# NagabhushanSN95/SimpleNeRF

Hardware: AMD Instinct MI355X
Metric: rays/sec (coarse+fine, 128+128 samples) (higher is better)
Workload: dtype f32; 1 GPU; headline: 1024 rays/GPU x (128 coarse + 128 fine -> 256 merged) samples, 8x256 coarse+fine MLPs, LLFF fern NDC rays, eval; rays_per_gpu=1024, samples=128+128, parallelism=ray-shard x1

## Files before the change

### simplenerf_amd/csrc/mlp_backward.hip

```cpp
#include "mlp_generic.h"
#include <algorithm>
#include <type_traits>

#include "mlp_device_f16.h"

namespace snerf {
int mlp_backward_chain_f16x3(const MlpPlan& plan, const ChainArgs& a, int products, hipStream_t stream);
int mlp_backward_chain_bf16(const MlpPlan& plan, const ChainArgs& a, hipStream_t stream);
}

namespace {

template <int U>
__device__ __forceinline__ void zero_acc(f32x16 (&acc)[U]) {
#pragma unroll
    for (int u = 0; u < U; ++u)
#pragma unroll
        for (int r = 0; r < 16; ++r) acc[u][r] = 0.0f;
}

template <int U>
__device__ __forceinline__ void load_relu_words(unsigned (&words)[U / 2], const unsigned* __restrict__ masks, int t0, int lane) {
#pragma unroll
    for (int p = 0; p < U / 2; ++p) words[p] = __builtin_nontemporal_load(masks + ((t0 >> 1) + p) * 64 + lane);
}
template <int U>
__device__ __forceinline__ void relu_backward(const f32x16 (&acc)[U], const unsigned (&words)[U / 2], float (&dy)[U * 16]) {
#pragma unroll
    for (int u = 0; u < U; u += 2)
#pragma unroll
        for (int r = 0; r < 32; ++r) dy[16 * u + r] = keep_if_bit(acc[u + (r >> 4)][r & 15], words[u >> 1], r);
}

template <int WT, int VT, bool VIEWDEP>
__global__ void __launch_bounds__(256, 1) mlp_backward_chain_kernel(ChainArgs a) {
    extern __shared__ __attribute__((aligned(16))) float lds[];
    const int lane = threadIdx.x & 63;
    const int wave = __builtin_amdgcn_readfirstlane(threadIdx.x >> 6);
    const int half = lane >> 5;
    SlabStream<WT> st;
    st.start(a.packed + a.dgrad_offset, lds, lane, wave);

    const long long block = (long long)blockIdx.x * 4 + wave;
    const long long first = block * 32 + (lane & 31);
    const bool live = first < a.total;
    const unsigned* masks = reinterpret_cast<const unsigned*>(a.acts + (block * a.act_rows + a.act_mask) * 32);
    float* grads = a.grads + block * a.grad_rows * 32;

    float dhead[4];
    dhead[0] = live && a.sigma[first] > 0.0f ? a.d_sigma[first] : 0.0f;
#pragma unroll
    for (int c = 0; c < 3; ++c) {
        const float col = live ? a.rgb[first * 3 + c] : 0.0f;
        dhead[c + 1] = live ? a.d_rgb[first * 3 + c] * (col * (1.0f - col)) : 0.0f;
    }
    if (half == 0) {
#pragma unroll
        for (int c = 0; c < 4; ++c) grads[(a.grad_head + c) * 32 + (lane & 31)] = dhead[c];
    }

    f32x16 acc[WT];
    zero_acc<WT>(acc);
    float dy[WT * 16];
    if (VIEWDEP) {
        const float* wv = a.packed + a.views_out_w;
        unsigned hv_bits[VT / 2];
#pragma unroll
        for (int p = 0; p < VT / 2; ++p) hv_bits[p] = masks[((a.depth * WT) / 2 + p) * 64 + lane];
        float dyv[VT * 16];
#pragma unroll
        for (int g = 0; g < VT * 4; ++g) {
            f32x4 w0 = *reinterpret_cast<const f32x4*>(wv + 0 * VT * 32 + 8 * g + 4 * half);
            f32x4 w1 = *reinterpret_cast<const f32x4*>(wv + 1 * VT * 32 + 8 * g + 4 * half);
            f32x4 w2 = *reinterpret_cast<const f32x4*>(wv + 2 * VT * 32 + 8 * g + 4 * half);
#pragma unroll
            for (int q = 0; q < 4; ++q) {
                const float v = fmaf(w2[q], dhead[3], fmaf(w1[q], dhead[2], w0[q] * dhead[1]));
                const int n = 4 * g + q;
                dyv[n] = (hv_bits[n >> 5] >> (n & 31)) & 1u ? v : 0.0f;
            }
        }
        store_acc_tile(dyv, grads + a.grad_yv * 32, lane);
        gemm_segment<WT, VT, WT>(acc, dyv, st);
        to_operand<WT, false>(acc, dy);
        store_acc_tile(dy, grads + a.grad_feature * 32, lane);
        zero_acc<WT>(acc);
        gemm_segment<WT, WT, WT>(acc, dy, st);
    }
    {
        const float* wo = a.packed + a.pts_out_w;
#pragma unroll
        for (int g = 0; g < WT * 4; ++g) {
            const f32x4 w0 = *reinterpret_cast<const f32x4*>(wo + 8 * g + 4 * half);
            f32x4 w1 = {0, 0, 0, 0}, w2 = {0, 0, 0, 0}, w3 = {0, 0, 0, 0};
            if (!VIEWDEP) {
                w1 = *reinterpret_cast<const f32x4*>(wo + 1 * WT * 32 + 8 * g + 4 * half);
                w2 = *reinterpret_cast<const f32x4*>(wo + 2 * WT * 32 + 8 * g + 4 * half);
                w3 = *reinterpret_cast<const f32x4*>(wo + 3 * WT * 32 + 8 * g + 4 * half);
            }
#pragma unroll
            for (int q = 0; q < 4; ++q) {
                float v = w0[q] * dhead[0];
                if (!VIEWDEP) v = fmaf(w3[q], dhead[3], fmaf(w2[q], dhead[2], fmaf(w1[q], dhead[1], v)));
                acc[g >> 2][4 * (g & 3) + q] += v;
            }
        }
    }
    unsigned relu_words[WT / 2];
    load_relu_words<WT>(relu_words, masks, (a.depth - 1) * WT, lane);
#pragma unroll 1
    for (int l = a.depth - 1; l >= 0; --l) {
        relu_backward<WT>(acc, relu_words, dy);
        if (l > 0) load_relu_words<WT>(relu_words, masks, (l - 1) * WT, lane);
        store_acc_tile(dy, grads + (l * a.width) * 32, lane);
        if (l == 0) break;
        zero_acc<WT>(acc);
        gemm_segment<WT, WT, WT>(acc, dy, st);
    }
    asm volatile("s_waitcnt vmcnt(0)" ::: "memory");
}

struct WgradJob {
    int dy_row0, out_rows, out_tiles;
    int x_row0, in_rows, in_tiles;
    int grad_rows, act_rows;
    int chunks;
    long long blocks;
    long long partial_off;
    long long bias_off;
    int w_param, w_ld, w_col;
    int b_param;
    int half;
    int dy_skip;
    int x_kind;
    int feat_lo, feat_hi;
    int x8;
    int x2_row0, x2_tiles;
    int launched, partial_ld, partial_col0;
};

__host__ __device__ inline int pe_position_feature(int p, int kind) {
    const int c = p & 15;
    const int n = 8 * (p >> 4) + 4 * (c >> 3) + (c & 3), h = (c >> 2) & 1;
    return snerf::pe_feature(n, h, kind == snerf::SEG_POINTS_PE ? snerf::kPointsPairs : snerf::kViewsPairs, 16);
}

constexpr int kRegionSlots = 64, kRegionWords = 128;
constexpr int kRegionTableFloat0 = 448;
__device__ __forceinline__ float region_max(const float* workspace, int region) {
    const unsigned w = reinterpret_cast<const unsigned*>(workspace)[kRegionTableFloat0 + (threadIdx.x & (kRegionSlots - 1)) * kRegionWords + region];
    float v = __uint_as_float(w);
#pragma unroll
    for (int off = 32; off > 0; off >>= 1) v = fmaxf(v, __shfl_xor(v, off, 64));
    return v;
}

__host__ __device__ inline float wgrad_scale(float max_abs) {
    if (!(max_abs > 0.0f) || !(max_abs < 3.0e38f)) return 1.0f;
    int e;
    frexpf(max_abs, &e);
    int shift = 10 - e;
    if (shift > 120) shift = 120;
    if (shift < -120) shift = -120;
    return ldexpf(1.0f, shift);
}

__device__ __forceinline__ void split_fragment(const float* __restrict__ row, int c0, int swz, float k, f16x8& hi, f16x8& lo,
                                               float& sum) {
    const f32x4 v0 = *reinterpret_cast<const f32x4*>(row + ((c0 ^ swz) << 2));
    const f32x4 v1 = *reinterpret_cast<const f32x4*>(row + (((c0 + 1) ^ swz) << 2));
    sum += (v0[0] + v0[1]) + (v0[2] + v0[3]) + (v1[0] + v1[1]) + (v1[2] + v1[3]);
    typedef float f32x2 __attribute__((ext_vector_type(2)));
    typedef _Float16 f16x2 __attribute__((ext_vector_type(2)));
#pragma unroll
    for (int j = 0; j < 4; j += 2) {
        const f32x2 a = f32x2{v0[j], v0[j + 1]} * k, b = f32x2{v1[j], v1[j + 1]} * k;
        const f16x2 ah = __builtin_convertvector(a, f16x2), bh = __builtin_convertvector(b, f16x2);
        const f16x2 al = __builtin_convertvector(a - __builtin_convertvector(ah, f32x2), f16x2);
        const f16x2 bl = __builtin_convertvector(b - __builtin_convertvector(bh, f32x2), f16x2);
        hi[j] = ah[0]; hi[j + 1] = ah[1]; lo[j] = al[0]; lo[j + 1] = al[1];
        hi[4 + j] = bh[0]; hi[5 + j] = bh[1]; lo[4 + j] = bl[0]; lo[5 + j] = bl[1];
    }
}

__device__ __forceinline__ void lds_dma_16(const float* src, const float* lds_dst) {
    const unsigned base = __builtin_amdgcn_readfirstlane(
        (unsigned)(size_t)(__attribute__((address_space(3))) const void*)lds_dst);
    asm volatile("s_mov_b32 m0, %0\n\ts_nop 0\n\tglobal_load_lds_dwordx4 %1, off nt" ::"s"(base), "v"(src) : "memory", "m0");
}

__device__ __forceinline__ void lds_dma_16_base(const void* uniform_base, unsigned lane_byte_offset, unsigned lds_byte_address) {
    asm volatile("s_mov_b32 m0, %0\n\ts_nop 0\n\tglobal_load_lds_dwordx4 %1, %2 nt" ::"s"(lds_byte_address), "v"(lane_byte_offset),
                 "s"(uniform_base)
                 : "memory", "m0");
}

constexpr int kMaxJobs = 16;
struct JobTable {
    int count;
    int wg_start[kMaxJobs + 1];
    WgradJob jobs[kMaxJobs];
};
struct GradPointers {
    float* p[40];
};

template <int NO, int NI, bool F16>
__global__ void __launch_bounds__(256, 1) wgrad_kernel(JobTable table, const float* __restrict__ grads,
                                                       const float* __restrict__ acts, float* __restrict__ partial,
                                                       const float* __restrict__ zeros) {
    extern __shared__ __attribute__((aligned(16))) float lds[];
    const int tid = threadIdx.x;
    const int lane = tid & 63;
    const int wave = __builtin_amdgcn_readfirstlane(tid >> 6);
    const int half = lane >> 5;
    int ji = 0;
    while (ji + 1 < table.count && (int)blockIdx.x >= table.wg_start[ji + 1]) ++ji;
    const WgradJob& job = table.jobs[ji];
    const int chunk = blockIdx.x - table.wg_start[ji];
    const int rows_dy = job.out_tiles * 32, rows_x = job.in_tiles * 32, rows = rows_dy + rows_x;
    const int wgrid_i = job.in_tiles / NI;
    const int wo = wave / wgrid_i, wi = wave - wo * wgrid_i;
    const bool active = wo * NO < job.out_tiles;
    const long long per = (job.blocks + job.chunks - 1) / job.chunks;
    const long long b0 = chunk * per, b1 = (b0 + per < job.blocks) ? b0 + per : job.blocks;

    f32x16 acc[NO][NI];
    float bsum[NO];
#pragma unroll
    for (int oo = 0; oo < NO; ++oo) {
        bsum[oo] = 0.0f;
#pragma unroll
        for (int ii = 0; ii < NI; ++ii)
#pragma unroll
            for (int r = 0; r < 16; ++r) acc[oo][ii][r] = 0.0f;
    }

    const int buf_floats = rows * 32;
    constexpr int kMaxSlots = 16;
    const int per_wave = rows >> 5;
    const char* slot_src[kMaxSlots];
    int slot_rows[kMaxSlots];
    const char* zero_page = reinterpret_cast<const char*>(zeros + 192);
    const long long dy_stride = (long long)job.grad_rows * 128, x_stride = (long long)job.act_rows * 128;
#pragma unroll
    for (int k = 0; k < kMaxSlots; ++k) {
        const int r0 = (wave + 4 * k) * 8;
        int real;
        const char* src;
        if (r0 < rows_dy) {
            real = job.out_rows - r0;
            src = reinterpret_cast<const char*>(grads) + (b0 * job.grad_rows + job.dy_row0 + r0) * 128;
        } else {
            real = job.in_rows - (r0 - rows_dy);
            src = reinterpret_cast<const char*>(acts) + (b0 * job.act_rows + job.x_row0 + (r0 - rows_dy)) * 128;
        }
        real = real < 0 ? 0 : (real > 8 ? 8 : real);
        slot_rows[k] = real;
        slot_src[k] = real > 0 ? src : zero_page;
    }
    const unsigned lane_off = (lane >> 3) * 128 + (((lane & 7) ^ ((4 * (wave & 1) + (lane >> 4)) & 7)) << 4);
    const unsigned lds_base = (unsigned)(size_t)(__attribute__((address_space(3))) const void*)lds;
    const bool all_full = job.out_rows == rows_dy && job.in_rows == rows_x;
    const int dy_slots = (rows_dy / 8 - wave + 3) >> 2;
    const char* dy_run = reinterpret_cast<const char*>(grads) + (b0 * job.grad_rows + job.dy_row0 + wave * 8) * 128;
    const char* x_run = reinterpret_cast<const char*>(acts) + (b0 * job.act_rows + job.x_row0 + wave * 8 - rows_dy) * 128;
    auto stage_next = [&](int buffer_floats) {
        if (all_full) {
#pragma unroll
            for (int k = 0; k < kMaxSlots; ++k)
                if (k < per_wave)
                    lds_dma_16_base(k < dy_slots ? dy_run : x_run, lane_off + k * 4096,
                                    lds_base + (unsigned)buffer_floats * 4 + (wave + 4 * k) * 1024);
            dy_run += dy_stride;
            x_run += x_stride;
            return;
        }
#pragma unroll
        for (int k = 0; k < kMaxSlots; ++k) {
            if (k < per_wave) {
                const unsigned dst = lds_base + (unsigned)buffer_floats * 4 + (wave + 4 * k) * 1024;
                const int real = slot_rows[k];
                if (real == 8 || real == 0) {
                    lds_dma_16_base(slot_src[k], real ? lane_off : lane * 16, dst);
                } else {
                    const char* p = (lane >> 3) < real ? slot_src[k] + lane_off : zero_page + lane * 16;
                    lds_dma_16(reinterpret_cast<const float*>(p), reinterpret_cast<const float*>(lds) + buffer_floats + (wave + 4 * k) * 256);
                }
                if (real) slot_src[k] += (wave + 4 * k) * 8 < rows_dy ? dy_stride : x_stride;
            }
        }
    };

    const int swz = ((lane & 31) >> 1) & 7;
    const int row_off = (lane & 31) * 32;
    const int a_base = wo * NO * 1024;
    const int b_base = rows_dy * 32 + wi * NI * 1024;

    const float gk = F16 ? wgrad_scale(region_max(zeros, job.dy_row0 / 32)) : 1.0f;
    if constexpr (F16) {
        struct SplitSet {
            f16x8 ah[NO], al[NO], bh[NI], bl[NI];
        };
        auto convert = [&](SplitSet& f, const float* buf, int kk, float counted) {
            const int c0 = 4 * kk + 2 * half;
            float unused = 0.0f;
#pragma unroll
            for (int oo = 0; oo < NO; ++oo) {
                float part = 0.0f;
                split_fragment(buf + a_base + oo * 1024 + row_off, c0, swz, gk, f.ah[oo], f.al[oo], part);
                bsum[oo] += part * counted;
            }
#pragma unroll
            for (int ii = 0; ii < NI; ++ii) split_fragment(buf + b_base + ii * 1024 + row_off, c0, swz, 1.0f, f.bh[ii], f.bl[ii], unused);
        };
        auto products = [&](const SplitSet& f) {
#pragma unroll
            for (int oo = 0; oo < NO; ++oo)
#pragma unroll
                for (int ii = 0; ii < NI; ++ii) {
                    acc[oo][ii] = __builtin_amdgcn_mfma_f32_32x32x16_f16(f.ah[oo], f.bh[ii], acc[oo][ii], 0, 0, 0);
                    acc[oo][ii] = __builtin_amdgcn_mfma_f32_32x32x16_f16(f.ah[oo], f.bl[ii], acc[oo][ii], 0, 0, 0);
                    acc[oo][ii] = __builtin_amdgcn_mfma_f32_32x32x16_f16(f.al[oo], f.bh[ii], acc[oo][ii], 0, 0, 0);
                }
        };
        const int nblocks = (int)(b1 - b0);
        SplitSet even, odd;
        if (nblocks > 0) {
            stage_next(0);
            if (nblocks > 1) stage_next(buf_floats);
            if (nblocks > 1) wait_vmcnt(per_wave < 63 ? per_wave : 63); else asm volatile("s_waitcnt vmcnt(0)" ::: "memory");
            __syncthreads();
            if (active) convert(even, lds, 0, 1.0f);
        }
        for (int n = 0; n < nblocks; ++n) {
            const float* cur = lds + (n & 1) * buf_floats;
            const float* nxt = lds + ((n + 1) & 1) * buf_floats;
            if (active) {
                products(even);
                convert(odd, cur, 1, 1.0f);
            }
            asm volatile("s_waitcnt vmcnt(0) lgkmcnt(0)" ::: "memory");
            __syncthreads();
            if (n + 2 < nblocks) stage_next((n & 1) * buf_floats);
            if (active) {
                products(odd);
                convert(even, n + 1 < nblocks ? nxt : cur, 0, n + 1 < nblocks ? 1.0f : 0.0f);
            }
        }
    } else {
    if (b0 < b1) stage_next(0);
    for (long long b = b0; b < b1; ++b) {
        asm volatile("s_waitcnt vmcnt(0)" ::: "memory");
        __syncthreads();
        const float* cur = lds + ((b - b0) & 1) * buf_floats;
        if (b + 1 < b1) stage_next((int)((b - b0 + 1) & 1) * buf_floats);
        if (active) {
#pragma unroll 1
            for (int g = 0; g < 4; ++g) {
                const int off = (((2 * g + half) ^ swz) << 2) + row_off;
                f32x4 av[NO], bv[NI];
#pragma unroll
                for (int oo = 0; oo < NO; ++oo) av[oo] = *reinterpret_cast<const f32x4*>(cur + a_base + oo * 1024 + off);
#pragma unroll
                for (int ii = 0; ii < NI; ++ii) bv[ii] = *reinterpret_cast<const f32x4*>(cur + b_base + ii * 1024 + off);
#pragma unroll
                for (int oo = 0; oo < NO; ++oo) {
#pragma unroll
                    for (int ii = 0; ii < NI; ++ii)
#pragma unroll
                        for (int q = 0; q < 4; ++q)
                            acc[oo][ii] = __builtin_amdgcn_mfma_f32_32x32x2f32(av[oo][q], bv[ii][q], acc[oo][ii], 0, 0, 0);
                    bsum[oo] += (av[oo][0] + av[oo][1]) + (av[oo][2] + av[oo][3]);
                }
            }
        }
    }
    }
    asm volatile("s_waitcnt vmcnt(0)" ::: "memory");
    if (!active) return;
    const int in_cols = job.in_tiles * 32;
    float* out = partial + job.partial_off + (long long)chunk * rows_dy * in_cols;
    float* bout = partial + job.bias_off + (long long)chunk * rows_dy;
#pragma unroll
    for (int oo = 0; oo < NO; ++oo) {
        const int o = wo * NO + oo;
#pragma unroll
        for (int ii = 0; ii < NI; ++ii) {
            const int i = wi * NI + ii;
#pragma unroll
            for (int r = 0; r < 16; ++r) {
                const int row = (r & 3) + 8 * (r >> 2) + 4 * half;
                out[(long long)(o * 32 + row) * in_cols + i * 32 + (lane & 31)] = acc[oo][ii][r];
            }
        }
        if (wi == 0) {
            const float sum = bsum[oo] + __shfl_xor(bsum[oo], 32, 64);
            if (half == 0) bout[o * 32 + lane] = sum;
        }
    }
}


typedef unsigned u32x2 __attribute__((ext_vector_type(2)));

__device__ __forceinline__ u32x2 lds_read_tr8(unsigned lds_byte_address, int byte_offset) {
    u32x2 v;
    asm volatile("ds_read_b64_tr_b8 %0, %1 offset:%2" : "=v"(v) : "v"(lds_byte_address), "i"(byte_offset) : "memory");
    return v;
}
__device__ __forceinline__ u32x2 lds_read_tr16(unsigned lds_byte_address, int byte_offset) {
    u32x2 v;
    asm volatile("ds_read_b64_tr_b16 %0, %1 offset:%2" : "=v"(v) : "v"(lds_byte_address), "i"(byte_offset) : "memory");
    return v;
}
template <typename T>
__device__ __forceinline__ void after_lds_wait(T& v) {
    asm volatile("" : "+v"(v));
}
union Frag16 {
// ... 805 lines not shown
```

### simplenerf_amd/csrc/mlp_device.h

```cpp
#pragma once
#include "mlp_plan.h"

typedef float f32x16 __attribute__((ext_vector_type(16)));
typedef float f32x4 __attribute__((ext_vector_type(4)));
typedef float f32x2 __attribute__((ext_vector_type(2)));

struct MlpArgs {
    const float* packed;
    const float* origins;
    const float* dirs;
    const float* view_dirs;
    const float* depths;
    const float* noise;
    float* sigma;
    float* rgb;
    long long total;
    int samples;
    int depth;
    int width;
    long long bias_offset, feature_bias, views_bias, pts_out_w, pts_out_b, views_out_w, views_out_b;
    float* acts;
    int act_rows, act_pev, act_h1, act_feature, act_hv, act_mask;
    int const_floats;
    float* visibility;
    const float* view_dirs2;
    float* visibility2;
    int num_other;
    int* range_flag;
    const int* weight_range;
};

struct ChainArgs {
    const float* packed;
    const float* acts;
    const float* sigma;
    const float* rgb;
    const float* d_sigma;
    const float* d_rgb;
    float* grads;
    long long total;
    int depth, width;
    long long dgrad_offset, pts_out_w, views_out_w;
    int act_rows, act_h1, act_hv, act_mask;
    int grad_rows, grad_feature, grad_yv, grad_head;
    unsigned* dy_max;
};

__host__ __device__ inline float renorm_factor(float max_abs) {
    if (!(max_abs > 0.0f) || !(max_abs < 3.0e38f)) return 1.0f;
    int e;
    frexpf(max_abs, &e);
    int shift = 4 - e;
    if (shift > 120) shift = 120;
    if (shift < -120) shift = -120;
    return ldexpf(1.0f, shift);
}

template <int N>
__device__ __forceinline__ void store_acc_tile(const float (&h)[N], float* __restrict__ tile, int lane) {
    const int j = lane & 31, half = lane >> 5;
#pragma unroll
    for (int n = 0; n < N; ++n) {
        const int f = 32 * (n >> 4) + (n & 3) + 8 * ((n & 15) >> 2) + 4 * half;
        __builtin_nontemporal_store(h[n], tile + f * 32 + j);
    }
}
template <int N>
__device__ __forceinline__ void load_acc_tile(float (&h)[N], const float* __restrict__ tile, int lane) {
    const int j = lane & 31, half = lane >> 5;
#pragma unroll
    for (int n = 0; n < N; ++n) {
        const int f = 32 * (n >> 4) + (n & 3) + 8 * ((n & 15) >> 2) + 4 * half;
        h[n] = tile[f * 32 + j];
    }
}
__device__ __forceinline__ float keep_if_bit(float v, unsigned word, int bit) {
    return __uint_as_float(__float_as_uint(v) & (unsigned)__builtin_amdgcn_sbfe((int)word, bit, 1));
}
__device__ __forceinline__ float keep_if_bit_2op(float v, unsigned word, int bit) {
    int k = __builtin_amdgcn_sbfe((int)word, bit, 1);
    asm("" : "+v"(k));
    return __uint_as_float(__float_as_uint(v) & (unsigned)k);
}
__device__ __forceinline__ unsigned positive_bits(unsigned m, float a, float b) {
    const f32x2 t = f32x2{0.0f, 0.0f} - f32x2{a, b};
    m = __builtin_amdgcn_alignbit(m, __float_as_uint(t[0]), 31);
    return __builtin_amdgcn_alignbit(m, __float_as_uint(t[1]), 31);
}
__device__ __forceinline__ unsigned relu_bits(const float* __restrict__ h) {
    unsigned m = 0;
#pragma unroll
    for (int r = 15; r >= 1; r -= 2) m = positive_bits(m, h[r], h[r - 1]);
    return m;
}
template <int N>
__device__ __forceinline__ void store_relu_masks(const float (&h)[N], unsigned* __restrict__ masks, int t0, int lane) {
#pragma unroll
    for (int u = 0; u < N / 16; u += 2)
        __builtin_nontemporal_store(relu_bits(h + 16 * u) | (relu_bits(h + 16 * (u + 1)) << 16), masks + ((t0 + u) >> 1) * 64 + lane);
}
template <int PAIRS, int NREG>
__device__ __forceinline__ void store_pe_tile(const float (&pe)[NREG], float* __restrict__ tile, int lane) {
    const int j = lane & 31, half = lane >> 5;
#pragma unroll
    for (int n = 0; n < NREG; ++n) {
        const int e0 = snerf::pe_feature(n, 0, PAIRS, 16), e1 = snerf::pe_feature(n, 1, PAIRS, 16);
        const int e = half ? e1 : e0;
        if (e >= 0) __builtin_nontemporal_store(pe[n], tile + e * 32 + j);
    }
}

template <int WT>
struct SlabStream {
    static constexpr int kBufFloats = WT * 1024;
    const float* cur;
    float* lds;
    int parity;
    int lane, wave;

    __device__ __forceinline__ void fetch(const float* src, float* dst) const {
#pragma unroll
        for (int i = 0; i < WT; ++i) {
            const int chunk = i * 4 + wave;
            __builtin_amdgcn_global_load_lds((const __attribute__((address_space(1))) void*)(src + chunk * 256 + lane * 4),
                                             (__attribute__((address_space(3))) void*)(dst + chunk * 256), 16, 0, 0);
        }
    }
    __device__ __forceinline__ void start(const float* first, float* lds_base, int lane_, int wave_) {
        cur = first; lds = lds_base; parity = 0; lane = lane_; wave = wave_;
        fetch(cur, lds);
    }
    template <int U>
    __device__ __forceinline__ const float* acquire() {
        asm volatile("s_waitcnt vmcnt(0)" ::: "memory");
        __syncthreads();
        const float* ready = lds + parity * kBufFloats;
        cur += U * 1024;
        parity ^= 1;
        return ready;
    }
    template <int I>
    __device__ __forceinline__ void fetch_piece() const {
        const int chunk = I * 4 + wave;
        __builtin_amdgcn_global_load_lds((const __attribute__((address_space(1))) void*)(cur + chunk * 256 + lane * 4),
                                         (__attribute__((address_space(3))) void*)(lds + parity * kBufFloats + chunk * 256),
                                         16, 0, 0);
    }
};

template <int I, int WT>
__device__ __forceinline__ void fetch_piece_if(const SlabStream<WT>& st) {
    if constexpr (I >= 0 && I < WT) st.template fetch_piece<I>();
}
template <int U, int WT, int EVERY>
__device__ __forceinline__ void constexpr_fetch(const SlabStream<WT>& st, int slot) {
#pragma unroll
    for (int i = 0; i < WT; ++i)
        if (slot == i * EVERY) {
            const int chunk = i * 4 + st.wave;
            __builtin_amdgcn_global_load_lds((const __attribute__((address_space(1))) void*)(st.cur + chunk * 256 + st.lane * 4),
                                             (__attribute__((address_space(3))) void*)(st.lds + st.parity * SlabStream<WT>::kBufFloats + chunk * 256),
                                             16, 0, 0);
        }
}
template <int WT, int DONE>
__device__ __forceinline__ void tail_fetch(const SlabStream<WT>& st) {
#pragma unroll
    for (int i = DONE; i < WT; ++i) {
        const int chunk = i * 4 + st.wave;
        __builtin_amdgcn_global_load_lds((const __attribute__((address_space(1))) void*)(st.cur + chunk * 256 + st.lane * 4),
                                         (__attribute__((address_space(3))) void*)(st.lds + st.parity * SlabStream<WT>::kBufFloats + chunk * 256),
                                         16, 0, 0);
    }
}

template <int U, int NSLAB, int WT, int NB>
__device__ __forceinline__ void gemm_segment(f32x16 (&acc)[U], const float (&b)[NB], SlabStream<WT>& st) {
    static_assert(NB >= NSLAB * 16, "B operand array too short");
    constexpr int kSlots = 4 * U;
    constexpr int kEvery = kSlots >= WT ? kSlots / WT : 1;
#pragma unroll
    for (int sl = 0; sl < NSLAB; ++sl) {
        const float* slab = st.template acquire<U>() + st.lane * 4;
#pragma unroll
        for (int g = 0; g < 4; ++g) {
#pragma unroll
            for (int u = 0; u < U; ++u) {
                const f32x4 a = *reinterpret_cast<const f32x4*>(slab + (g * U + u) * 256);
#pragma unroll
                for (int q = 0; q < 4; ++q)
                    acc[u] = __builtin_amdgcn_mfma_f32_32x32x2f32(a[q], b[sl * 16 + g * 4 + q], acc[u], 0, 0, 0);
                constexpr_fetch<U, WT, kEvery>(st, g * U + u);
            }
        }
        if (kSlots < WT) tail_fetch<WT, kSlots>(st);
    }
}

template <int U, int NB>
__device__ __forceinline__ void gemm_resident_slab(f32x16 (&acc)[U], const float (&b)[NB], const float* slab) {
    static_assert(NB >= 16, "B operand array too short");
#pragma unroll
    for (int g = 0; g < 4; ++g) {
#pragma unroll
        for (int u = 0; u < U; ++u) {
            const f32x4 a = *reinterpret_cast<const f32x4*>(slab + (g * U + u) * 256);
#pragma unroll
            for (int q = 0; q < 4; ++q) acc[u] = __builtin_amdgcn_mfma_f32_32x32x2f32(a[q], b[g * 4 + q], acc[u], 0, 0, 0);
        }
    }
}

template <int U>
__device__ __forceinline__ void load_bias(f32x16 (&acc)[U], const float* __restrict__ bias, int half) {
#pragma unroll
    for (int u = 0; u < U; ++u) {
#pragma unroll
        for (int g = 0; g < 4; ++g) {
            const f32x4 v = *reinterpret_cast<const f32x4*>(bias + 32 * u + 8 * g + 4 * half);
#pragma unroll
            for (int q = 0; q < 4; ++q) acc[u][4 * g + q] = v[q];
        }
    }
}

template <int U, bool RELU>
__device__ __forceinline__ void to_operand(const f32x16 (&acc)[U], float (&h)[U * 16]) {
#pragma unroll
    for (int u = 0; u < U; ++u)
#pragma unroll
        for (int r = 0; r < 16; ++r) h[16 * u + r] = RELU ? fmaxf(acc[u][r], 0.0f) : acc[u][r];
}

template <int N>
__device__ __forceinline__ float head_dot(const float (&h)[N], const float* __restrict__ w, int half) {
    float s = 0.0f;
#pragma unroll
    for (int g = 0; g < N / 4; ++g) {
        const f32x4 v = *reinterpret_cast<const f32x4*>(w + 8 * g + 4 * half);
#pragma unroll
        for (int q = 0; q < 4; ++q) s = fmaf(v[q], h[4 * g + q], s);
    }
    return s + __shfl_xor(s, 32, 64);
}

__device__ __forceinline__ float sigmoidf(float x) { return __fdiv_rn(1.0f, 1.0f + expf(-x)); }

__device__ __forceinline__ f32x2 opaque_pair(float v) {
    f32x2 p = {v, v};
    asm volatile("" : "+v"(p));
    return p;
}

template <bool PAIRED = false>
__device__ __forceinline__ void sincos_turns(double turns, float& s, float& c) {
    const double f = turns - rint(turns);
    const double q = rint(4.0 * f);
    const double g = f - 0.25 * q;
    const float th = (float)(g * 6.283185307179586476925);
    float t2 = th * th, t2c = t2;
    if constexpr (PAIRED) {
        const f32x2 both = opaque_pair(t2);
        t2 = both.x; t2c = both.y;
    }
    float sp = fmaf(t2, 2.7557319e-6f, -1.9841270e-4f);
    sp = fmaf(sp, t2, 8.3333333e-3f);
    sp = fmaf(sp, t2, -1.6666667e-1f);
    sp = fmaf(th * t2, sp, th);
    float cp = fmaf(t2c, -2.7557319e-7f, 2.4801587e-5f);
    cp = fmaf(cp, t2c, -1.3888889e-3f);
    cp = fmaf(cp, t2c, 4.1666667e-2f);
    cp = fmaf(cp, t2c, -0.5f);
    cp = fmaf(cp, t2c, 1.0f);
    const int qi = ((int)q) & 3;
    const float s0 = (qi & 1) ? cp : sp;
    const float c0 = (qi & 1) ? sp : cp;
    s = (qi >= 2) ? -s0 : s0;
    c = (qi == 1 || qi == 2) ? -c0 : c0;
}

template <int PAIRS, int NREG, bool PAIRED = false>
__device__ __forceinline__ void encode(const float (&x)[3], int half, float (&pe)[NREG]) {
    constexpr double kInvTwoPi = 0.15915494309189533576888;
    const double r0 = (double)x[0] * kInvTwoPi, r1 = (double)x[1] * kInvTwoPi, r2 = (double)x[2] * kInvTwoPi;
#pragma unroll
    for (int m = 0; m < PAIRS / 2; ++m) {
        constexpr int dummy = 0;
        (void)dummy;
        const int c0 = 2 * m, c1 = 2 * m + 1;
        const int d0 = c0 % 3, d1 = c1 % 3;
        const double a0 = d0 == 0 ? r0 : (d0 == 1 ? r1 : r2);
        const double a1 = d1 == 0 ? r0 : (d1 == 1 ? r1 : r2);
        const double f0 = (double)(1 << (c0 / 3)), f1 = (double)(1 << (c1 / 3));
        const double turns = half ? a1 * f1 : a0 * f0;
        sincos_turns<PAIRED>(turns, pe[2 * m], pe[2 * m + 1]);
    }
    pe[PAIRS] = half ? x[2] : x[0];
    pe[PAIRS + 1] = half ? 0.0f : x[1];
#pragma unroll
    for (int n = PAIRS + 2; n < NREG; ++n) pe[n] = 0.0f;
}
```

### simplenerf_amd/csrc/mlp_forward_body.h

```cpp
#pragma once
#include "mlp_device.h"

namespace {

template <int WT, int VT, bool VIEWDEP, bool SIGMA_PE, bool STORE, bool VIS = false>
__device__ __forceinline__ void mlp_forward_body(const MlpArgs& a, long long block, float* lds) {
    static_assert(!VIS || VIEWDEP, "the visibility row belongs to the views head");
    const int lane = threadIdx.x & 63;
    const int wave = __builtin_amdgcn_readfirstlane(threadIdx.x >> 6);
    const int half = lane >> 5;

    SlabStream<WT> st;
    st.start(a.packed, lds, lane, wave);
    float* consts = lds + 2 * SlabStream<WT>::kBufFloats;
    for (int i = threadIdx.x * 4; i < a.const_floats; i += 256 * 4)
        *reinterpret_cast<f32x4*>(consts + i) = *reinterpret_cast<const f32x4*>(a.packed + a.bias_offset + i);
    __syncthreads();

    const long long first = (block * 4 + wave) * 32 + (lane & 31);
    const bool live = first < a.total;
    const long long g = live ? first : a.total - 1;
    const long long ray = g / a.samples;
    const float z = a.depths[g];
    float x[3];
#pragma unroll
    for (int k = 0; k < 3; ++k) x[k] = a.origins[ray * 3 + k] + a.dirs[ray * 3 + k] * z;

    float pe[snerf::kPointsKSteps];
    encode<snerf::kPointsPairs, snerf::kPointsKSteps>(x, half, pe);
    float pev[snerf::kViewsKSteps];
    if (VIEWDEP) {
        float v[3];
#pragma unroll
        for (int k = 0; k < 3; ++k) v[k] = a.view_dirs[ray * 3 + k];
        encode<snerf::kViewsPairs, snerf::kViewsKSteps>(v, half, pev);
    }

    float* tile = nullptr;
    unsigned* masks = nullptr;
    if (STORE) {
        tile = a.acts + (block * 4 + wave) * a.act_rows * 32;
        masks = reinterpret_cast<unsigned*>(tile + a.act_mask * 32);
        store_pe_tile<snerf::kPointsPairs, snerf::kPointsKSteps>(pe, tile, lane);
        if (VIEWDEP) store_pe_tile<snerf::kViewsPairs, snerf::kViewsKSteps>(pev, tile + a.act_pev * 32, lane);
    }

    const float* bias = consts;
    f32x16 acc[WT];
    float h[WT * 16];
    load_bias<WT>(acc, bias, half);
    gemm_segment<WT, 2, WT>(acc, pe, st);
    to_operand<WT, true>(acc, h);
    if (STORE) {
        store_acc_tile(h, tile + a.act_h1 * 32, lane);
        store_relu_masks(h, masks, 0, lane);
    }
#pragma unroll 1
    for (int l = 1; l < a.depth; ++l) {
        load_bias<WT>(acc, bias + (long long)l * a.width, half);
        if (l == 5) gemm_segment<WT, 2, WT>(acc, pe, st);
        gemm_segment<WT, WT, WT>(acc, h, st);
        to_operand<WT, true>(acc, h);
        if (STORE) {
            store_acc_tile(h, tile + (a.act_h1 + l * a.width) * 32, lane);
            store_relu_masks(h, masks, l * WT, lane);
        }
    }

    const float* wout = consts + (a.pts_out_w - a.bias_offset);
    const float* bout = consts + (a.pts_out_b - a.bias_offset);
    float sigma = head_dot<WT * 16>(h, wout, half) + bout[0];
    if (a.noise) sigma += a.noise[g];
    sigma = fmaxf(sigma, 0.0f);
    float rgb[3];
    if (!VIEWDEP) {
#pragma unroll
        for (int c = 0; c < 3; ++c) rgb[c] = sigmoidf(head_dot<WT * 16>(h, wout + (c + 1) * WT * 32, half) + bout[c + 1]);
    } else {
        load_bias<WT>(acc, consts + (a.feature_bias - a.bias_offset), half);
        gemm_segment<WT, WT, WT>(acc, h, st);
        to_operand<WT, false>(acc, h);
        if (STORE) store_acc_tile(h, tile + a.act_feature * 32, lane);
        f32x16 accv[VT];
        load_bias<VT>(accv, consts + (a.views_bias - a.bias_offset), half);
        gemm_segment<VT, WT, WT>(accv, h, st);
        if (SIGMA_PE) gemm_segment<VT, 2, WT>(accv, pe, st);
        f32x16 accv_base[VT];
        const float* view_slab = nullptr;
        if constexpr (VIS) {
#pragma unroll
            for (int u = 0; u < VT; ++u) accv_base[u] = accv[u];
            view_slab = st.template acquire<VT>() + lane * 4;
            gemm_resident_slab<VT>(accv, pev, view_slab);
        } else {
            gemm_segment<VT, 1, WT>(accv, pev, st);
        }
        float hv[VT * 16];
        to_operand<VT, true>(accv, hv);
        if (STORE) {
            store_acc_tile(hv, tile + a.act_hv * 32, lane);
            store_relu_masks(hv, masks, a.depth * WT, lane);
        }
        const float* wv = consts + (a.views_out_w - a.bias_offset);
        const float* bv = consts + (a.views_out_b - a.bias_offset);
#pragma unroll
        for (int c = 0; c < 3; ++c) rgb[c] = sigmoidf(head_dot<VT * 16>(hv, wv + c * VT * 32, half) + bv[c]);
        if constexpr (VIS) {
            const float vis = sigmoidf(head_dot<VT * 16>(hv, wv + 3 * VT * 32, half) + bv[3]);
            if (a.visibility && live && half == 0) a.visibility[first] = vis;
#pragma unroll 1
            for (int k = 0; k < a.num_other; ++k) {
                float v2[3], pev2[snerf::kViewsKSteps];
#pragma unroll
                for (int c = 0; c < 3; ++c) v2[c] = a.view_dirs2[(g * a.num_other + k) * 3 + c];
                encode<snerf::kViewsPairs, snerf::kViewsKSteps>(v2, half, pev2);
                f32x16 acc2[VT];
#pragma unroll
                for (int u = 0; u < VT; ++u) acc2[u] = accv_base[u];
                gemm_resident_slab<VT>(acc2, pev2, view_slab);
                float hv2[VT * 16];
                to_operand<VT, true>(acc2, hv2);
                const float vis2 = sigmoidf(head_dot<VT * 16>(hv2, wv + 3 * VT * 32, half) + bv[3]);
                if (live && half == 0) a.visibility2[first * a.num_other + k] = vis2;
            }
        }
    }

    asm volatile("s_waitcnt vmcnt(0)" ::: "memory");
    if (live && half == 0) {
        a.sigma[first] = sigma;
        a.rgb[first * 3 + 0] = rgb[0];
        a.rgb[first * 3 + 1] = rgb[1];
        a.rgb[first * 3 + 2] = rgb[2];
    }
}

constexpr int kMaxConstFloats = 5120;

}
```

Measured before the change: 311,900 rays/s.

## Interleave activation and gradient tile stores into the MFMA slab loop

The separate activation/gradient tile stores and ReLU mask stores that ran after each layer's GEMM are folded into the gemm_segment loop, issued at fixed MFMA slots of the next layer's GEMM that consumes that operand. Slab acquisition now waits on a counted vmcnt instead of draining to zero, so the in-flight stores do not stall the weight-slab pipeline. This aims to hide global store latency behind matrix math. In exchange it adds fragile hard-coded vmcnt bookkeeping and store schedules that only hold for specific segment shapes.

```diff
diff --git a/simplenerf_amd/csrc/mlp_backward.hip b/simplenerf_amd/csrc/mlp_backward.hip
--- a/simplenerf_amd/csrc/mlp_backward.hip
+++ b/simplenerf_amd/csrc/mlp_backward.hip
@@ -46,6 +46,7 @@
     const bool live = first < a.total;
     const unsigned* masks = reinterpret_cast<const unsigned*>(a.acts + (block * a.act_rows + a.act_mask) * 32);
     float* grads = a.grads + block * a.grad_rows * 32;
+    const unsigned lane_row = 128 * half + (lane & 31);
 
     float dhead[4];
     dhead[0] = live && a.sigma[first] > 0.0f ? a.d_sigma[first] : 0.0f;
@@ -80,12 +81,10 @@
                 dyv[n] = (hv_bits[n >> 5] >> (n & 31)) & 1u ? v : 0.0f;
             }
         }
-        store_acc_tile(dyv, grads + a.grad_yv * 32, lane);
-        gemm_segment<WT, VT, WT>(acc, dyv, st);
+        gemm_segment<WT, VT, WT, kStoreOperand>(acc, dyv, st, grads + a.grad_yv * 32, nullptr, lane_row);
         to_operand<WT, false>(acc, dy);
-        store_acc_tile(dy, grads + a.grad_feature * 32, lane);
         zero_acc<WT>(acc);
-        gemm_segment<WT, WT, WT>(acc, dy, st);
+        gemm_segment<WT, WT, WT, kStoreOperand>(acc, dy, st, grads + a.grad_feature * 32, nullptr, lane_row);
     }
     {
         const float* wo = a.packed + a.pts_out_w;
@@ -112,10 +111,12 @@
     for (int l = a.depth - 1; l >= 0; --l) {
         relu_backward<WT>(acc, relu_words, dy);
         if (l > 0) load_relu_words<WT>(relu_words, masks, (l - 1) * WT, lane);
-        store_acc_tile(dy, grads + (l * a.width) * 32, lane);
-        if (l == 0) break;
+        if (l == 0) {
+            store_acc_tile(dy, grads, lane);
+            break;
+        }
         zero_acc<WT>(acc);
-        gemm_segment<WT, WT, WT>(acc, dy, st);
+        gemm_segment<WT, WT, WT, kStoreOperand>(acc, dy, st, grads + (l * a.width) * 32, nullptr, lane_row);
     }
     asm volatile("s_waitcnt vmcnt(0)" ::: "memory");
 }
diff --git a/simplenerf_amd/csrc/mlp_device.h b/simplenerf_amd/csrc/mlp_device.h
--- a/simplenerf_amd/csrc/mlp_device.h
+++ b/simplenerf_amd/csrc/mlp_device.h
@@ -117,6 +117,7 @@
     float* lds;
     int parity;
     int lane, wave;
+    int younger;
 
     __device__ __forceinline__ void fetch(const float* src, float* dst) const {
 #pragma unroll
@@ -127,7 +128,7 @@
         }
     }
     __device__ __forceinline__ void start(const float* first, float* lds_base, int lane_, int wave_) {
-        cur = first; lds = lds_base; parity = 0; lane = lane_; wave = wave_;
+        cur = first; lds = lds_base; parity = 0; lane = lane_; wave = wave_; younger = 0;
         fetch(cur, lds);
     }
     template <int U>
@@ -139,6 +140,31 @@
         parity ^= 1;
         return ready;
     }
+    template <int U, int N>
+    __device__ __forceinline__ const float* acquire_counted() {
+        asm volatile("s_waitcnt vmcnt(%0)" ::"n"(N) : "memory");
+        return handed_over<U>();
+    }
+    template <int U>
+    __device__ __forceinline__ const float* acquire_counted_first() {
+        const int n = younger;
+        younger = 0;
+        if (n == 20) asm volatile("s_waitcnt vmcnt(20)" ::: "memory");
+        else if (n == 18) asm volatile("s_waitcnt vmcnt(18)" ::: "memory");
+        else if (n == 16) asm volatile("s_waitcnt vmcnt(16)" ::: "memory");
+        else asm volatile("s_waitcnt vmcnt(0)" ::: "memory");
+        return handed_over<U>();
+    }
+    template <int U>
+    __device__ __forceinline__ const float* handed_over() {
+        asm volatile("s_waitcnt lgkmcnt(0)" ::: "memory");
+        __builtin_amdgcn_s_barrier();
+        asm volatile("" ::: "memory");
+        const float* ready = lds + parity * kBufFloats;
+        cur += U * 1024;
+        parity ^= 1;
+        return ready;
+    }
     template <int I>
     __device__ __forceinline__ void fetch_piece() const {
         const int chunk = I * 4 + wave;
@@ -174,14 +200,29 @@
     }
 }
 
-template <int U, int NSLAB, int WT, int NB>
-__device__ __forceinline__ void gemm_segment(f32x16 (&acc)[U], const float (&b)[NB], SlabStream<WT>& st) {
+enum { kPlainSegment = 0, kCountedSegment = 1, kStoreOperand = 2, kStoreOperandAndMasks = 3 };
+
+template <int U, int NSLAB, int WT, int MODE = kPlainSegment, int NB>
+__device__ __forceinline__ void gemm_segment(f32x16 (&acc)[U], const float (&b)[NB], SlabStream<WT>& st, float* rows = nullptr,
+                                             unsigned* words = nullptr, unsigned lane_row = 0) {
     static_assert(NB >= NSLAB * 16, "B operand array too short");
+    constexpr bool kStores = MODE >= kStoreOperand;
     constexpr int kSlots = 4 * U;
-    constexpr int kEvery = kSlots >= WT ? kSlots / WT : 1;
+    constexpr int kHalf = kSlots / 2;
+    constexpr int kEvery = kStores ? kHalf / WT : (kSlots >= WT ? kSlots / WT : 1);
+    constexpr int kPerSlot = kStores ? 16 / kHalf : 1;
+    constexpr int kWords = MODE == kStoreOperandAndMasks ? NSLAB / 2 : 0;
+    static_assert(!kStores || (NB == NSLAB * 16 && kHalf >= WT && kHalf % WT == 0 && kHalf <= 16 && 16 % kHalf == 0 && kWords <= kHalf),
+                  "no store schedule for this segment shape");
 #pragma unroll
     for (int sl = 0; sl < NSLAB; ++sl) {
-        const float* slab = st.template acquire<U>() + st.lane * 4;
+        const float* slab;
+        if constexpr (MODE == kPlainSegment) {
+            slab = st.template acquire<U>() + st.lane * 4;
+        } else {
+            if (sl == 0) slab = st.template acquire_counted_first<U>() + st.lane * 4;
+            else slab = st.template acquire_counted<U, kStores ? 16 : 0>() + st.lane * 4;
+        }
 #pragma unroll
         for (int g = 0; g < 4; ++g) {
 #pragma unroll
@@ -191,10 +232,22 @@
                 for (int q = 0; q < 4; ++q)
                     acc[u] = __builtin_amdgcn_mfma_f32_32x32x2f32(a[q], b[sl * 16 + g * 4 + q], acc[u], 0, 0, 0);
                 constexpr_fetch<U, WT, kEvery>(st, g * U + u);
+                if constexpr (kStores) {
+                    const int slot = g * U + u;
+#pragma unroll
+                    for (int n = 0; n < 16; ++n)
+                        if (slot == kHalf + n / kPerSlot)
+                            __builtin_nontemporal_store(b[16 * sl + n], rows + (32 * sl + (n & 3) + 8 * (n >> 2)) * 32 + lane_row);
+#pragma unroll
+                    for (int p = 0; p < kWords; ++p)
+                        if (sl == NSLAB - 1 && slot == kHalf + p)
+                            __builtin_nontemporal_store(relu_bits(b + 32 * p) | (relu_bits(b + 32 * p + 16) << 16), words + p * 64 + st.lane);
+                }
             }
         }
         if (kSlots < WT) tail_fetch<WT, kSlots>(st);
     }
+    if constexpr (kStores) st.younger = 16 + kWords;
 }
 
 template <int U, int NB>
diff --git a/simplenerf_amd/csrc/mlp_forward_body.h b/simplenerf_amd/csrc/mlp_forward_body.h
--- a/simplenerf_amd/csrc/mlp_forward_body.h
+++ b/simplenerf_amd/csrc/mlp_forward_body.h
@@ -36,6 +36,10 @@
         encode<snerf::kViewsPairs, snerf::kViewsKSteps>(v, half, pev);
     }
 
+    constexpr int kSegment = STORE ? kCountedSegment : kPlainSegment;
+    constexpr int kSegmentKeep = STORE ? kStoreOperand : kPlainSegment;
+    constexpr int kSegmentKeepRelu = STORE ? kStoreOperandAndMasks : kPlainSegment;
+    const unsigned lane_row = 128 * half + (lane & 31);
     float* tile = nullptr;
     unsigned* masks = nullptr;
     if (STORE) {
@@ -49,22 +53,15 @@
     f32x16 acc[WT];
     float h[WT * 16];
     load_bias<WT>(acc, bias, half);
-    gemm_segment<WT, 2, WT>(acc, pe, st);
+    gemm_segment<WT, 2, WT, kSegment>(acc, pe, st);
     to_operand<WT, true>(acc, h);
-    if (STORE) {
-        store_acc_tile(h, tile + a.act_h1 * 32, lane);
-        store_relu_masks(h, masks, 0, lane);
-    }
 #pragma unroll 1
     for (int l = 1; l < a.depth; ++l) {
         load_bias<WT>(acc, bias + (long long)l * a.width, half);
-        if (l == 5) gemm_segment<WT, 2, WT>(acc, pe, st);
-        gemm_segment<WT, WT, WT>(acc, h, st);
+        if (l == 5) gemm_segment<WT, 2, WT, kSegment>(acc, pe, st);
+        gemm_segment<WT, WT, WT, kSegmentKeepRelu>(acc, h, st, tile + (a.act_h1 + (l - 1) * a.width) * 32, masks + ((l - 1) * WT / 2) * 64,
+                                                   lane_row);
         to_operand<WT, true>(acc, h);
-        if (STORE) {
-            store_acc_tile(h, tile + (a.act_h1 + l * a.width) * 32, lane);
-            store_relu_masks(h, masks, l * WT, lane);
-        }
     }
 
     const float* wout = consts + (a.pts_out_w - a.bias_offset);
@@ -74,26 +71,31 @@
     sigma = fmaxf(sigma, 0.0f);
     float rgb[3];
     if (!VIEWDEP) {
+        if (STORE) {
+            store_acc_tile(h, tile + (a.act_h1 + (a.depth - 1) * a.width) * 32, lane);
+            store_relu_masks(h, masks, (a.depth - 1) * WT, lane);
+        }
 #pragma unroll
         for (int c = 0; c < 3; ++c) rgb[c] = sigmoidf(head_dot<WT * 16>(h, wout + (c + 1) * WT * 32, half) + bout[c + 1]);
     } else {
         load_bias<WT>(acc, consts + (a.feature_bias - a.bias_offset), half);
-        gemm_segment<WT, WT, WT>(acc, h, st);
+        gemm_segment<WT, WT, WT, kSegmentKeepRelu>(acc, h, st, tile + (a.act_h1 + (a.depth - 1) * a.width) * 32,
+                                                   masks + ((a.depth - 1) * WT / 2) * 64, lane_row);
         to_operand<WT, false>(acc, h);
-        if (STORE) store_acc_tile(h, tile + a.act_feature * 32, lane);
         f32x16 accv[VT];
         load_bias<VT>(accv, consts + (a.views_bias - a.bias_offset), half);
-        gemm_segment<VT, WT, WT>(accv, h, st);
-        if (SIGMA_PE) gemm_segment<VT, 2, WT>(accv, pe, st);
+        gemm_segment<VT, WT, WT, kSegmentKeep>(accv, h, st, tile + a.act_feature * 32, nullptr, lane_row);
+        if (SIGMA_PE) gemm_segment<VT, 2, WT, kSegment>(accv, pe, st);
         f32x16 accv_base[VT];
         const float* view_slab = nullptr;
         if constexpr (VIS) {
 #pragma unroll
             for (int u = 0; u < VT; ++u) accv_base[u] = accv[u];
-            view_slab = st.template acquire<VT>() + lane * 4;
+            if constexpr (STORE) view_slab = st.template acquire_counted_first<VT>() + lane * 4;
+            else view_slab = st.template acquire<VT>() + lane * 4;
             gemm_resident_slab<VT>(accv, pev, view_slab);
         } else {
-            gemm_segment<VT, 1, WT>(accv, pev, st);
+            gemm_segment<VT, 1, WT, kSegment>(accv, pev, st);
         }
         float hv[VT * 16];
         to_operand<VT, true>(accv, hv);
```

New measurement: 312,000 rays/s, median of 2. About the same (+0.0%).
